# anitasyang/Laplace-GNN

Measured on AMD Instinct MI355X. Metric: la.fit() samples/sec (GCN, KFAC), higher is better.
Workload: dtype f32; 1 GPU; arxiv-shaped 2-layer GCN, hessian_structure=kron (BASELINE configs[2]); num_nodes=169343, nnz=2501719, features=128, hidden=256, classes=40, n_train=90941, batch_size=10000, batches=10, parallelism=dp1 ((batch, class) units, contiguous balanced runs)

## Files before the change

### include/laplace_gnn_hip.h

```cpp
#ifndef LAPLACE_GNN_HIP_H
#define LAPLACE_GNN_HIP_H

#include <stdint.h>

#ifdef __cplusplus
extern "C" {
#endif

#define LGNN_ABI_VERSION 1

#if defined(__GNUC__)
#define LGNN_API __attribute__((visibility("default")))
#else
#define LGNN_API
#endif

#define LGNN_KIND_GCN 0
#define LGNN_KIND_SAGE 1

#define LGNN_ACT_RELU 0
#define LGNN_ACT_TANH 1

#define LGNN_NORM_NONE 0
#define LGNN_NORM_LAYER 1
// ... 25 lines not shown
LGNN_API int lgnn_is_symmetric(const lgnn_ctx* h);

LGNN_API int lgnn_export_adj(const lgnn_ctx* h, int64_t* rows, int64_t* cols, void* stream);
LGNN_API int lgnn_adj_to_edge_index(const lgnn_ctx* h, int64_t* edge_index_out, int64_t* num_out, void* stream);
LGNN_API int lgnn_update_adjacency(lgnn_ctx* h, const int64_t* rows, const int64_t* cols, const uint8_t* state,
                                   int64_t num_flips, void* stream);
LGNN_API int lgnn_export_propagation(const lgnn_ctx* h, int64_t* rows, int64_t* cols, float* vals, void* stream);

LGNN_API int lgnn_bind_model(lgnn_ctx* h, int num_layers, const int64_t* dims ,
                    const float* const* weights ,
                    const float* const* biases , const float* X,
                    int activation, int likelihood);
LGNN_API int lgnn_bind_extras(lgnn_ctx* h, const float* const* res_weights, const float* const* res_biases, int norm_kind,
                     const float* const* norm_weight, const float* const* norm_bias, const float* const* norm_mean,
                     const float* const* norm_var, float norm_eps);
LGNN_API int lgnn_invalidate(lgnn_ctx* h);
LGNN_API int64_t lgnn_device_bytes(const lgnn_ctx* h);
LGNN_API int lgnn_set_workspace_limit(lgnn_ctx* h, int64_t bytes);

LGNN_API int lgnn_forward(lgnn_ctx* h, const int64_t* idx, int64_t M, float* out , void* stream);
LGNN_API int lgnn_forward_all(lgnn_ctx* h, float* out , void* stream);

#define LGNN_SAMPLED_SOFTMAX 1u
LGNN_API int lgnn_sampled_forward(lgnn_ctx* h, const int64_t* idx, int64_t M, const float* theta ,
                                  int64_t S, uint32_t flags , float* out ,
                                  void* stream);

LGNN_API int lgnn_train_forward(lgnn_ctx* h, const int64_t* idx, int64_t M, const uint8_t* const* drop_masks ,
                                float drop_scale, float* out , void* stream);
LGNN_API int lgnn_train_backward(lgnn_ctx* h, const float* grad_out , float* const* grad_W, float* const* grad_b,
                                 float* const* grad_res_W, float* const* grad_res_b, float* const* grad_norm_w,
                                 float* const* grad_norm_b, void* stream);

LGNN_API int lgnn_kfac_accumulate(lgnn_ctx* h, const int64_t* idx, const void* y, int64_t M, int64_t n_train,
                         uint32_t flags, float* const* A_out ,
                         float* const* B_out , float* loss_out,
                         void* stream);

LGNN_API int lgnn_kfac_accumulate_classes(lgnn_ctx* h, const int64_t* idx, const void* y, int64_t M, int64_t n_train,
                                 uint32_t flags, int64_t class_begin, int64_t class_end,
                                 float* const* A_out, float* const* B_out, float* loss_out, void* stream);

LGNN_API int lgnn_kfac_accumulate_share(lgnn_ctx* h, const int64_t* idx, const void* y, int64_t M, int64_t n_train,
                               uint32_t flags, int64_t part_begin, int64_t part_end, int64_t part_count,
                               float* const* A_out, float* const* B_out, float* loss_out, void* stream);

LGNN_API int lgnn_kfac_accumulate_fisher(lgnn_ctx* h, const int64_t* idx, const void* y_seed, const void* y_loss, int64_t M,
                                int64_t n_train, uint32_t flags, float resid_scale, float b_scale, float* const* A_out,
                                float* const* B_out, float* loss_out, void* stream);
LGNN_API int lgnn_ef_accumulate(lgnn_ctx* h, const int64_t* idx, const void* y_seed, const void* y_loss, int64_t M,
                       float resid_scale, float scale, float* diag_out, float* full_out, float* grads_out,
                       float* loss_out, void* stream);

LGNN_API int lgnn_kfac_plan(int kind, int num_layers, const int64_t* dims , int64_t num_nodes, int64_t nnz,
                   int activation, uint32_t flags, int64_t workspace_limit, int64_t* out );

LGNN_API int lgnn_diag_accumulate(lgnn_ctx* h, const int64_t* idx, const void* y, int64_t M, uint32_t flags,
                         float* diag_out , float* loss_out, void* stream);

LGNN_API int lgnn_full_accumulate(lgnn_ctx* h, const int64_t* idx, const void* y, int64_t M, float* H_out, float* loss_out,
                         void* stream);

LGNN_API int lgnn_lastlayer_full_accumulate(lgnn_ctx* h, const int64_t* idx, const void* y, int64_t M,
                                   float* H_out, float* loss_out, void* stream);

LGNN_API int lgnn_lastlayer_features(lgnn_ctx* h, const int64_t* idx, int64_t M, float* phi_out, float* f_out, void* stream);

LGNN_API int lgnn_lastlayer_pairs_accumulate(lgnn_ctx* h, const int64_t* idx, const void* y, int64_t M, float* S_pairs,
                                    float* Sb_pairs, float* loss_out, void* stream);
LGNN_API int lgnn_lastlayer_pairs_place(lgnn_ctx* h, const float* S_pairs, const float* Sb_pairs, float* H_out, void* stream);

LGNN_API int lgnn_lastlayer_kron_accumulate(lgnn_ctx* h, const int64_t* idx, const void* y, int64_t M, int64_t n_train,
                                   uint32_t flags, float* A_out, float* B_out, float* Bb_out, float* loss_out, void* stream);
LGNN_API int lgnn_lastlayer_diag_accumulate(lgnn_ctx* h, const int64_t* idx, const void* y, int64_t M, float* diag_out,
                                   float* loss_out, void* stream);

LGNN_API int lgnn_check_async_errors(lgnn_ctx* h, void* stream);
LGNN_API int lgnn_peek_async_errors(lgnn_ctx* h);

LGNN_API int lgnn_kfac_batch_tag(lgnn_ctx* h, uint64_t tag);
LGNN_API int lgnn_batch_cache_drop(lgnn_ctx* h, uint64_t tag);
LGNN_API int lgnn_batch_cache_stats(const lgnn_ctx* h, int64_t* out);

LGNN_API int lgnn_enable_kernel_timing(lgnn_ctx* h, int enable);
LGNN_API int lgnn_kernel_timing_read(lgnn_ctx* h, int64_t* launches, double* total_ms, int64_t* planes);
LGNN_API int lgnn_kernel_timing_launches(lgnn_ctx* h, double* ms_out, int64_t capacity, int64_t* launches);

LGNN_API int lgnn_jacobians(lgnn_ctx* h, const int64_t* idx, int64_t M, float* J, float* f_out, void* stream);

LGNN_API int lgnn_jacobians_subset(lgnn_ctx* h, const int64_t* idx, int64_t M, const int64_t* subnet, int64_t S, float* J,
                          float* f_out, void* stream);
LGNN_API int lgnn_subnet_full_accumulate(lgnn_ctx* h, const int64_t* idx, const void* y, int64_t M, const int64_t* subnet,
                                int64_t S, float* H_out, float* loss_out, void* stream);

#define LGNN_GP_INDEPENDENT 1
#define LGNN_GP_MATCHED 2
#define LGNN_GP_FROM_JACOBIANS 4
LGNN_API int lgnn_gp_kernel(lgnn_ctx* h, const int64_t* idx_a, int64_t Ma, const int64_t* idx_b, int64_t Mb, int flags,
                            float* K, int64_t ldk, void* stream);
LGNN_API int lgnn_gp_jvp(lgnn_ctx* h, const int64_t* idx, int64_t M, const float* v, float* out, void* stream);

LGNN_API int lgnn_kfac_adjgrad_batch(lgnn_ctx* h, const int64_t* idx, const void* y, int64_t M, uint32_t flags,
                            const float* const* gamma_B , float loss_scale,
                            float* grad_P, float* out_bar, const int32_t* cand_a, const int32_t* cand_b, int64_t num_cand,
                            float* grad_cand, void* stream);
LGNN_API int lgnn_adjgrad_finish(lgnn_ctx* h, const float* out_bar, const float* const* gamma_A ,
                        float a_scale, float* grad_P, float* grad_adj, const int32_t* cand_a, const int32_t* cand_b,
                        int64_t num_cand, float* grad_cand, float* grad_cand_adj, void* stream);

LGNN_API int lgnn_diag_adjgrad_batch(lgnn_ctx* h, const int64_t* idx, const void* y, int64_t M, const float* gamma,
                            float loss_scale, float* grad_P, float* out_bar, float* h1_bar, float* e_bar,
                            const int32_t* cand_a, const int32_t* cand_b, int64_t num_cand, float* grad_cand, void* stream);
LGNN_API int lgnn_diag_adjgrad_finish(lgnn_ctx* h, const float* out_bar, const float* h1_bar, const float* e_bar, float* grad_P,
                             float* grad_adj, const int32_t* cand_a, const int32_t* cand_b, int64_t num_cand,
                             float* grad_cand, float* grad_cand_adj, void* stream);

LGNN_API int lgnn_full_adjgrad_batch(lgnn_ctx* h, const int64_t* idx, const void* y, int64_t M, const float* Gamma,
                            float loss_scale, float* grad_P, float* out_bar, float* h1_bar, float* e_bar,
                            const int32_t* cand_a, const int32_t* cand_b, int64_t num_cand, float* grad_cand, void* stream);
LGNN_API int lgnn_full_directions(lgnn_ctx* h, const int64_t* idx, int64_t M, const float* Gamma, float* K_out, float* R_out,
                         void* stream);

LGNN_API int lgnn_kfac_adjgrad_batch_dense(lgnn_ctx* h, const int64_t* idx, const void* y, int64_t M, uint32_t flags,
                                  const float* const* gamma_B , float loss_scale,
                                  float* out_bar, float* grad_adj_dense, void* stream);
LGNN_API int lgnn_adjgrad_finish_dense(lgnn_ctx* h, const float* out_bar, const float* const* gamma_A, float a_scale,
                              float* grad_adj_dense, void* stream);
LGNN_API int lgnn_diag_adjgrad_batch_dense(lgnn_ctx* h, const int64_t* idx, const void* y, int64_t M, const float* gamma,
                                  float loss_scale, float* out_bar, float* h1_bar, float* e_bar, float* grad_adj_dense,
                                  void* stream);
LGNN_API int lgnn_diag_adjgrad_finish_dense(lgnn_ctx* h, const float* out_bar, const float* h1_bar, const float* e_bar,
                                   float* grad_adj_dense, void* stream);

LGNN_API int lgnn_lora_threshold(lgnn_ctx* h, const int32_t* base_rowptr, const int32_t* base_col, const float* lora_A,
                                 const float* lora_B, int64_t r, float scaling, float threshold, int symmetric,
                                 int64_t* num_flips, void* stream);
LGNN_API int lgnn_lora_grad(lgnn_ctx* h, const float* grad_adj_dense, const float* lora_A, const float* lora_B, int64_t r,
                            float scaling, float* grad_A, float* grad_B, void* stream);

LGNN_API int lgnn_glm_variance(lgnn_ctx* h, const int64_t* idx, int64_t M, const float* QA0, const float* QB0, const float* S0,
                      const float* QA1, const float* S1, const float* QB1sq, const float* kappa, float* f_mu,
                      float* f_var_diag, void* stream);
LGNN_API int lgnn_glm_variance_mapped(lgnn_ctx* h, const int64_t* idx, int64_t M, const float* W1m, int64_t Cm,
                             const float* QA0, const float* QB0, const float* S0, const float* QA1, const float* S1,
                             const float* QB1sq, const float* kappa, float* f_mu, float* var_mapped, void* stream);

LGNN_API int lgnn_glm_variance_ext(lgnn_ctx* h, const int64_t* idx, int64_t M, const float* W1m, int64_t Cm,
                          const float* QA0, const float* QB0, const float* S0, const float* QA1, const float* S1,
                          const float* QB1sq, const float* kappa, const float* QAr, const float* QBr, const float* Sr,
                          float* f_mu, float* f_var, void* stream);

LGNN_API int lgnn_symeig_batched(float* A, int64_t n, int64_t batch, float* W, int32_t* info, void* stream);

LGNN_API int lgnn_knn(const float* X, int64_t N, int64_t F, int64_t ld, int k, int32_t* nbr, float* dist,
                      int64_t* num_fallback, void* stream);

#ifdef __cplusplus
}
#endif
#endif
```

### laplace-gnn_amd/_lib.py

```python
from __future__ import annotations

import ctypes as C
import os

_HERE = os.path.dirname(os.path.abspath(__file__))
LIB_PATH = os.path.join(_HERE, os.environ.get("LGNN_LIB_DIR", "lib"), "liblaplace_gnn_hip.so")

KIND_GCN, KIND_SAGE = 0, 1
ACT_RELU, ACT_TANH = 0, 1
LIK_CLASSIFICATION, LIK_REGRESSION = 0, 1
NORM_NONE, NORM_LAYER, NORM_BATCH = 0, 1, 2
FLAG_FORK_EXACT_SEED, FLAG_NO_FUSE, FLAG_NO_PATHS, FLAG_FORCE_PATHS = 1, 2, 4, 8
GP_INDEPENDENT, GP_MATCHED, GP_FROM_JACOBIANS = 1, 2, 4
SAMPLED_SOFTMAX = 1

_vp, _i64, _i32, _u32 = C.c_void_p, C.c_int64, C.c_int, C.c_uint32
_pp = C.POINTER(C.c_void_p)
SIGNATURES = {
    "lgnn_abi_version": (_i32, []),
    "lgnn_last_error": (C.c_char_p, []),
    "lgnn_create": (_i32, [_pp, _i64, _vp, _i64, _i32, _i32, _vp]),
    "lgnn_destroy": (None, [_vp]),
    "lgnn_nnz": (_i64, [_vp]),
    "lgnn_num_nodes": (_i64, [_vp]),
    "lgnn_is_symmetric": (_i32, [_vp]),
    "lgnn_num_long_rows": (_i64, [_vp]),
    "lgnn_kfac_last_route": (_i32, [_vp]),
    "lgnn_kfac_last_top": (_i32, [_vp]),
    "lgnn_kfac_last_top_kernel": (_i32, [_vp]),
    "lgnn_export_adj": (_i32, [_vp, _vp, _vp, _vp]),
    "lgnn_update_adjacency": (_i32, [_vp, _vp, _vp, _vp, _i64, _vp]),
    "lgnn_adj_to_edge_index": (_i32, [_vp, _vp, C.POINTER(_i64), _vp]),
    "lgnn_export_propagation": (_i32, [_vp, _vp, _vp, _vp, _vp]),
    "lgnn_bind_model": (_i32, [_vp, _i32, C.POINTER(_i64), _pp, _pp, _vp, _i32, _i32]),
    "lgnn_bind_extras": (_i32, [_vp, _pp, _pp, _i32, _pp, _pp, _pp, _pp, C.c_float]),
    "lgnn_invalidate": (_i32, [_vp]),
    "lgnn_device_bytes": (_i64, [_vp]),
    "lgnn_set_workspace_limit": (_i32, [_vp, _i64]),
    "lgnn_forward": (_i32, [_vp, _vp, _i64, _vp, _vp]),
    "lgnn_forward_all": (_i32, [_vp, _vp, _vp]),
    "lgnn_sampled_forward": (_i32, [_vp, _vp, _i64, _vp, _i64, _u32, _vp, _vp]),
    "lgnn_train_forward": (_i32, [_vp, _vp, _i64, _pp, C.c_float, _vp, _vp]),
    "lgnn_train_backward": (_i32, [_vp, _vp, _pp, _pp, _pp, _pp, _pp, _pp, _vp]),
    "lgnn_kfac_accumulate": (_i32, [_vp, _vp, _vp, _i64, _i64, _u32, _pp, _pp, _vp, _vp]),
    "lgnn_kfac_accumulate_classes": (_i32, [_vp, _vp, _vp, _i64, _i64, _u32, _i64, _i64, _pp, _pp, _vp, _vp]),
    "lgnn_kfac_accumulate_share": (_i32, [_vp, _vp, _vp, _i64, _i64, _u32, _i64, _i64, _i64, _pp, _pp, _vp, _vp]),
    "lgnn_kfac_accumulate_fisher": (_i32, [_vp, _vp, _vp, _vp, _i64, _i64, _u32, C.c_float, C.c_float, _pp, _pp, _vp, _vp]),
    "lgnn_ef_accumulate": (_i32, [_vp, _vp, _vp, _vp, _i64, C.c_float, C.c_float, _vp, _vp, _vp, _vp, _vp]),
    "lgnn_kfac_plan": (_i32, [_i32, _i32, C.POINTER(_i64), _i64, _i64, _i32, _u32, _i64, C.POINTER(_i64)]),
    "lgnn_diag_accumulate": (_i32, [_vp, _vp, _vp, _i64, _u32, _vp, _vp, _vp]),
    "lgnn_full_accumulate": (_i32, [_vp, _vp, _vp, _i64, _vp, _vp, _vp]),
    "lgnn_lastlayer_full_accumulate": (_i32, [_vp, _vp, _vp, _i64, _vp, _vp, _vp]),
    "lgnn_lastlayer_features": (_i32, [_vp, _vp, _i64, _vp, _vp, _vp]),
    "lgnn_lastlayer_pairs_accumulate": (_i32, [_vp, _vp, _vp, _i64, _vp, _vp, _vp, _vp]),
    "lgnn_lastlayer_pairs_place": (_i32, [_vp, _vp, _vp, _vp, _vp]),
    "lgnn_lastlayer_kron_accumulate": (_i32, [_vp, _vp, _vp, _i64, _i64, _u32, _vp, _vp, _vp, _vp, _vp]),
    "lgnn_lastlayer_diag_accumulate": (_i32, [_vp, _vp, _vp, _i64, _vp, _vp, _vp]),
    "lgnn_check_async_errors": (_i32, [_vp, _vp]),
    "lgnn_peek_async_errors": (_i32, [_vp]),
    "lgnn_kfac_batch_tag": (_i32, [_vp, C.c_uint64]),
    "lgnn_batch_cache_drop": (_i32, [_vp, C.c_uint64]),
    "lgnn_batch_cache_stats": (_i32, [_vp, C.POINTER(_i64)]),
    "lgnn_enable_kernel_timing": (_i32, [_vp, _i32]),
    "lgnn_kernel_timing_read": (_i32, [_vp, C.POINTER(_i64), C.POINTER(C.c_double), C.POINTER(_i64)]),
    "lgnn_kernel_timing_launches": (_i32, [_vp, _vp, _i64, _vp]),
    "lgnn_kfac_adjgrad_batch": (_i32, [_vp, _vp, _vp, _i64, _u32, _pp, C.c_float, _vp, _vp, _vp, _vp, _i64, _vp, _vp]),
    "lgnn_adjgrad_finish": (_i32, [_vp, _vp, _pp, C.c_float, _vp, _vp, _vp, _vp, _i64, _vp, _vp, _vp]),
    "lgnn_diag_adjgrad_batch": (_i32, [_vp, _vp, _vp, _i64, _vp, C.c_float, _vp, _vp, _vp, _vp, _vp, _vp, _i64, _vp, _vp]),
    "lgnn_diag_adjgrad_finish": (_i32, [_vp, _vp, _vp, _vp, _vp, _vp, _vp, _vp, _i64, _vp, _vp, _vp]),
    "lgnn_full_adjgrad_batch": (_i32, [_vp, _vp, _vp, _i64, _vp, C.c_float, _vp, _vp, _vp, _vp, _vp, _vp, _i64, _vp, _vp]),
    "lgnn_full_directions": (_i32, [_vp, _vp, _i64, _vp, _vp, _vp, _vp]),
    "lgnn_kfac_adjgrad_batch_dense": (_i32, [_vp, _vp, _vp, _i64, _u32, _pp, C.c_float, _vp, _vp, _vp]),
    "lgnn_adjgrad_finish_dense": (_i32, [_vp, _vp, _pp, C.c_float, _vp, _vp]),
    "lgnn_diag_adjgrad_batch_dense": (_i32, [_vp, _vp, _vp, _i64, _vp, C.c_float, _vp, _vp, _vp, _vp, _vp]),
    "lgnn_diag_adjgrad_finish_dense": (_i32, [_vp, _vp, _vp, _vp, _vp, _vp]),
    "lgnn_lora_threshold": (_i32, [_vp, _vp, _vp, _vp, _vp, _i64, C.c_float, C.c_float, _i32, C.POINTER(_i64), _vp]),
    "lgnn_lora_grad": (_i32, [_vp, _vp, _vp, _vp, _i64, C.c_float, _vp, _vp, _vp]),
    "lgnn_glm_variance": (_i32, [_vp, _vp, _i64, _vp, _vp, _vp, _vp, _vp, _vp, _vp, _vp, _vp, _vp]),
    "lgnn_glm_variance_mapped": (_i32, [_vp, _vp, _i64, _vp, _i64, _vp, _vp, _vp, _vp, _vp, _vp, _vp, _vp, _vp, _vp]),
    "lgnn_glm_variance_ext": (_i32, [_vp, _vp, _i64, _vp, _i64, _vp, _vp, _vp, _vp, _vp, _vp, _vp, _vp, _vp, _vp, _vp, _vp,
                                     _vp]),
    "lgnn_symeig_batched": (_i32, [_vp, _i64, _i64, _vp, _vp, _vp]),
    "lgnn_jacobians": (_i32, [_vp, _vp, _i64, _vp, _vp, _vp]),
    "lgnn_jacobians_subset": (_i32, [_vp, _vp, _i64, _vp, _i64, _vp, _vp, _vp]),
    "lgnn_subnet_full_accumulate": (_i32, [_vp, _vp, _vp, _i64, _vp, _i64, _vp, _vp, _vp]),
    "lgnn_gp_kernel": (_i32, [_vp, _vp, _i64, _vp, _i64, _i32, _vp, _i64, _vp]),
    "lgnn_gp_jvp": (_i32, [_vp, _vp, _i64, _vp, _vp, _vp]),
    "lgnn_knn": (_i32, [_vp, _i64, _i64, _i64, _i32, _vp, _vp, C.POINTER(_i64), _vp]),
}

_lib = None


class HipLibraryError(RuntimeError):
    pass


def load():
    global _lib
    if _lib is not None:
        return _lib
    if not os.path.exists(LIB_PATH):
        raise HipLibraryError(
            f"{LIB_PATH} is missing: build it with `python -c 'import __graft_entry__ as g; g.build()'` "
            "(or `make -C laplace-gnn_amd/csrc`).  There is no CPU fallback."
        )
    lib = C.CDLL(LIB_PATH)
    for name, (res, args) in SIGNATURES.items():
        fn = getattr(lib, name)
        fn.restype, fn.argtypes = res, args
    if lib.lgnn_abi_version() != 1:
        raise HipLibraryError("ABI version mismatch between _lib.py and liblaplace_gnn_hip.so")
    _lib = lib
    return lib


def check(rc: int, what: str):
    if rc != 0:
        msg = load().lgnn_last_error().decode("utf-8", "replace")
        raise HipLibraryError(f"{what} failed (rc={rc}): {msg}")


def ptr_array(ptrs):
    arr = (C.c_void_p * len(ptrs))(*ptrs)
    return arr
```

### laplace-gnn_amd/csrc/eigh.hip

```cpp
#include <cstdio>

#include <rocsolver/rocsolver.h>

#include "gram256.h"
#include "lgnn_internal.h"

namespace lgnn {
namespace {
rocblas_handle g_handle = nullptr;
rocblas_handle g_eig_handle = nullptr;
struct EighScratch {
  DevBuf e_large;
  DevBuf e;
  DevBuf v;
  DevBuf tau;
  DevBuf d;
  DevBuf z;
  DevBuf info;
};
EighScratch& scratch() {
  static auto* s = new EighScratch;
  return *s;
}

constexpr int kBranches = 8;
rocblas_handle g_bh[kBranches] = {};
hipStream_t g_side[kBranches] = {};
hipEvent_t g_fork = nullptr, g_join[kBranches] = {};
constexpr int TN = 256;

__device__ __forceinline__ float wsum64(float v) {
#pragma unroll
  for (int o = 32; o > 0; o >>= 1) v += __shfl_xor(v, o);
  return v;
}

__global__ __launch_bounds__(1024) void tridiag256_kernel(const float* __restrict__ A, int n, float* __restrict__ D,
                                                          float* __restrict__ E, float* __restrict__ V,
                                                          float* __restrict__ tau, int nfull, int off, int vld) {
  __shared__ __attribute__((aligned(16))) float xs[TN], vs[TN], ps[TN], ws[TN];
  const int tid = threadIdx.x, lane = tid & 63, r = tid >> 2, q = tid & 3;
  const int64_t b = blockIdx.x;
  const float* __restrict__ Ab = A + b * int64_t(nfull) * nfull + int64_t(off) * nfull + off;
  float* __restrict__ Db = D + b * int64_t(nfull) + off;
  float* __restrict__ Eb = E + b * int64_t(nfull) + off;
  float* __restrict__ Vb = V + b * int64_t(nfull) * vld + int64_t(off) * vld + off;
  float* __restrict__ tb = tau + b * int64_t(nfull) + off;
  float a[64];
#pragma unroll
  for (int g = 0; g < 16; ++g)
#pragma unroll
    for (int i = 0; i < 4; ++i) {
      const int c = 16 * g + 4 * q + i;
      a[4 * g + i] = (r < n && c < n) ? Ab[int64_t(r) * nfull + c] : 0.f;
    }
  for (int k = 0; k < n - 1; ++k) {
    const int g0 = (k + 1) >> 4;
    if (r == k) {
#pragma unroll
      for (int g = 0; g < 16; ++g)
        *reinterpret_cast<float4*>(&xs[16 * g + 4 * q]) = make_float4(a[4 * g], a[4 * g + 1], a[4 * g + 2], a[4 * g + 3]);
    }
    __syncthreads();
    float sg = 0.f;
#pragma unroll
    for (int j = 0; j < 4; ++j) {
      const int c = lane + 64 * j;
      const float x = xs[c];
      sg += c > k + 1 ? x * x : 0.f;
    }
    sg = wsum64(sg);
    const float alpha = xs[k + 1];
    if (tid == 0) Db[k] = xs[k];
    if (sg == 0.f) {
      if (tid == 0) { Eb[k] = alpha; tb[k] = 0.f; }
      __syncthreads();
      continue;
    }
    const float nrm = sqrtf(alpha * alpha + sg);
    const float beta = alpha >= 0.f ? -nrm : nrm;
    const float t = (beta - alpha) / beta;
    const float inv = 1.f / (alpha - beta);
    if (tid < TN) {
      const float v = tid <= k ? 0.f : (tid == k + 1 ? 1.f : xs[tid] * inv);
      vs[tid] = v;
      Vb[int64_t(k) * vld + tid] = v;
    }
    if (tid == 0) { Eb[k] = beta; tb[k] = t; }
    __syncthreads();
    if (r > k) {
      float part = 0.f;
#pragma unroll
      for (int g = 0; g < 16; ++g)
        if (g >= g0) {
          const float4 v4 = *reinterpret_cast<const float4*>(&vs[16 * g + 4 * q]);
          part = fmaf(a[4 * g], v4.x, part); part = fmaf(a[4 * g + 1], v4.y, part);
          part = fmaf(a[4 * g + 2], v4.z, part); part = fmaf(a[4 * g + 3], v4.w, part);
        }
      part += __shfl_xor(part, 1);
      part += __shfl_xor(part, 2);
      if (q == 0) ps[r] = t * part;
    } else if (q == 0) {
      ps[r] = 0.f;
    }
    __syncthreads();
    float ds = 0.f;
#pragma unroll
    for (int j = 0; j < 4; ++j) ds += ps[lane + 64 * j] * vs[lane + 64 * j];
    ds = wsum64(ds);
    const float hd = 0.5f * t * ds;
    if (tid < TN) ws[tid] = ps[tid] - hd * vs[tid];
    __syncthreads();
    if (r > k) {
      const float vr = vs[r], wr = ws[r];
#pragma unroll
      for (int g = 0; g < 16; ++g)
        if (g >= g0) {
          const float4 v4 = *reinterpret_cast<const float4*>(&vs[16 * g + 4 * q]);
          const float4 w4 = *reinterpret_cast<const float4*>(&ws[16 * g + 4 * q]);
          a[4 * g] -= vr * w4.x + wr * v4.x; a[4 * g + 1] -= vr * w4.y + wr * v4.y;
          a[4 * g + 2] -= vr * w4.z + wr * v4.z; a[4 * g + 3] -= vr * w4.w + wr * v4.w;
        }
    }
  }
  if (r == n - 1) {
#pragma unroll
    for (int g = 0; g < 16; ++g)
      *reinterpret_cast<float4*>(&xs[16 * g + 4 * q]) = make_float4(a[4 * g], a[4 * g + 1], a[4 * g + 2], a[4 * g + 3]);
  }
  __syncthreads();
  if (tid == 0) { Db[n - 1] = xs[n - 1]; Eb[n - 1] = 0.f; tb[n - 1] = 0.f; }
}

__global__ __launch_bounds__(256) void backtransform_kernel(const float* __restrict__ Z, int n, const float* __restrict__ V,
                                                            const float* __restrict__ tau, const float* __restrict__ lam,
                                                            const int32_t* __restrict__ info_in, float* __restrict__ out,
                                                            float* __restrict__ W, int32_t* __restrict__ info) {
  const int lane = threadIdx.x & 63;
  const int j = blockIdx.x * 4 + (threadIdx.x >> 6);
  const int64_t b = blockIdx.y;
  if (j >= n) return;
  if (lane == 0) {
    W[b * n + j] = lam[b * n + j];
    if (j == 0) info[b] = info_in[b];
  }
  const float* __restrict__ zr = Z + (b * n + j) * int64_t(n);
  float* __restrict__ orow = out + (b * n + j) * int64_t(n);
  const float* __restrict__ Vb = V + b * int64_t(n) * TN;
  const float* __restrict__ tb = tau + b * int64_t(n);
  float z[4];
#pragma unroll
  for (int i = 0; i < 4; ++i) z[i] = 4 * lane + i < n ? zr[4 * lane + i] : 0.f;
  for (int k = n - 2; k >= 0; --k) {
    const float t = tb[k];
    if (t == 0.f) continue;
    const float4 v = *reinterpret_cast<const float4*>(Vb + int64_t(k) * TN + 4 * lane);
    float d = v.x * z[0] + v.y * z[1] + v.z * z[2] + v.w * z[3];
    d = wsum64(d) * t;
    z[0] -= d * v.x; z[1] -= d * v.y; z[2] -= d * v.z; z[3] -= d * v.w;
  }
#pragma unroll
  for (int i = 0; i < 4; ++i)
    if (4 * lane + i < n) orow[4 * lane + i] = z[i];
}

constexpr int SNB = 32;
constexpr int SRG = 8;
__global__ __launch_bounds__(1024) void tridiag_stream_kernel(float* __restrict__ A, int n, int ncols, float* __restrict__ D,
                                                              float* __restrict__ E, float* __restrict__ V,
                                                              float* __restrict__ tau) {
// ... 40 lines not shown
        const float x = c < n ? xs[c] : 0.f;
        sg += c > k + 1 ? x * x : 0.f;
      }
      sg = wsum64(sg);
      const float alpha = xs[k + 1];
      float t = 0.f, beta = alpha, inv = 0.f;
      if (sg != 0.f) {
        const float nrm = sqrtf(alpha * alpha + sg);
        beta = alpha >= 0.f ? -nrm : nrm;
        t = (beta - alpha) / beta;
        inv = 1.f / (alpha - beta);
      }
      if (tid < n) {
        const float v = (sg == 0.f || tid <= k) ? 0.f : (tid == k + 1 ? 1.f : xs[tid] * inv);
        vs[tid] = v;
        Vp[j * n + tid] = v;
        Vb[int64_t(k) * n + tid] = v;
      }
      if (tid == 0) { Db[k] = xs[k]; Eb[k] = beta; tb[k] = t; }
      __syncthreads();
      if (sg == 0.f) {
        if (tid < n) Wp[j * n + tid] = 0.f;
        __syncthreads();
        continue;
      }
      {
        float4 acc = make_float4(0.f, 0.f, 0.f, 0.f);
        if (c4 + 3 > k && c4 < n) {
          int r = k + 1 + rg;
          for (; r + 7 * SRG < n; r += 8 * SRG) {
            float4 a[8];
#pragma unroll
            for (int u = 0; u < 8; ++u) a[u] = *reinterpret_cast<const float4*>(Ab + int64_t(r + u * SRG) * n + c4);
#pragma unroll
            for (int u = 0; u < 8; ++u) {
              const float vv = vs[r + u * SRG];
              acc.x += a[u].x * vv; acc.y += a[u].y * vv; acc.z += a[u].z * vv; acc.w += a[u].w * vv;
            }
          }
          for (; r < n; r += SRG) {
            const float4 a0 = *reinterpret_cast<const float4*>(Ab + int64_t(r) * n + c4);
            const float v0 = vs[r];
            acc.x += a0.x * v0; acc.y += a0.y * v0; acc.z += a0.z * v0; acc.w += a0.w * v0;
          }
        }
        if (c4 < n) *reinterpret_cast<float4*>(pp + rg * n + c4) = acc;
        for (int i = wave; i < j; i += 16) {
          float s1 = 0.f, s2 = 0.f;
          for (int q = 0; q < per_lane; ++q) {
            const int c = lane + 64 * q;
            if (c < n) { const float v = vs[c]; s1 += Wp[i * n + c] * v; s2 += Vp[i * n + c] * v; }
          }
          s1 = wsum64(s1); s2 = wsum64(s2);
          if (lane == 0) { tv[i] = s1; tw[i] = s2; }
        }
      }
      __syncthreads();
      if (tid < n) {
        float p = 0.f;
        if (tid > k) {
#pragma unroll
          for (int g = 0; g < SRG; ++g) p += pp[g * n + tid];
          float p2 = 0.f;
#pragma unroll 4
          for (int i = 0; i < j; ++i) {
            p -= Vp[i * n + tid] * tv[i];
            p2 += Wp[i * n + tid] * tw[i];
          }
          p -= p2;
        }
        ps[tid] = t * p;
      }
      __syncthreads();
      float ds = 0.f;
      for (int q = 0; q < per_lane; ++q) {
        const int c = lane + 64 * q;
        if (c < n) ds += ps[c] * vs[c];
      }
      ds = wsum64(ds);
      const float hd = 0.5f * t * ds;
      if (tid < n) Wp[j * n + tid] = ps[tid] - hd * vs[tid];
      __syncthreads();
    }
    const int kb = k0 + jn;
    if (jn < SNB) {
      for (int q = tid; q < (SNB - jn) * n; q += 1024) { Vp[jn * n + q] = 0.f; Wp[jn * n + q] = 0.f; }
      __syncthreads();
    }
    {
      const int base = kb & ~31;
      const int nt = (n - base + 31) >> 5;
      const int l31 = lane & 31, lhi = lane >> 5;
      for (int tile = wave; tile < nt * nt; tile += 16) {
        const int tr = tile / nt, tc = tile - tr * nt;
        const int row = base + 32 * tr + l31, col = base + 32 * tc + l31;
        const int rr = row < n ? row : n - 1, cc = col < n ? col : n - 1;
        f32x16 acc;
#pragma unroll
        for (int q = 0; q < 16; ++q) acc[q] = 0.f;
#pragma unroll 8
        for (int kk = 0; kk < SNB / 2; ++kk) {
          const int i = 2 * kk + lhi;
          acc = __builtin_amdgcn_mfma_f32_32x32x2f32(Vp[i * n + rr], Wp[i * n + cc], acc, 0, 0, 0);
          acc = __builtin_amdgcn_mfma_f32_32x32x2f32(Wp[i * n + rr], Vp[i * n + cc], acc, 0, 0, 0);
        }
        if (col < n) {
#pragma unroll
          for (int q = 0; q < 16; ++q) {
            const int r = base + 32 * tr + (q & 3) + 8 * (q >> 2) + 4 * lhi;
            if (r < n) Ab[int64_t(r) * n + col] -= acc[q];
          }
        }
      }
    }
    __syncthreads();
  }
}

__global__ __launch_bounds__(256) void backtransform512_kernel(const float* __restrict__ Z, int n, const float* __restrict__ V,
                                                               const float* __restrict__ tau, const float* __restrict__ lam,
                                                               const int32_t* __restrict__ info_in, float* __restrict__ out,
                                                               float* __restrict__ W, int32_t* __restrict__ info) {
  const int lane = threadIdx.x & 63;
  const int j = blockIdx.x * 4 + (threadIdx.x >> 6);
  const int64_t b = blockIdx.y;
  if (j >= n) return;
  if (lane == 0) {
    W[b * n + j] = lam[b * n + j];
    if (j == 0) info[b] = info_in[b];
  }
  const float* __restrict__ zr = Z + (b * n + j) * int64_t(n);
  float* __restrict__ orow = out + (b * n + j) * int64_t(n);
  const float* __restrict__ Vb = V + b * int64_t(n) * n;
  const float* __restrict__ tb = tau + b * int64_t(n);
  const bool hi = 256 + 4 * lane < n;
  const bool lo = 4 * lane < n;
  float4 z0 = lo ? *reinterpret_cast<const float4*>(zr + 4 * lane) : make_float4(0.f, 0.f, 0.f, 0.f);
  float4 z1 = hi ? *reinterpret_cast<const float4*>(zr + 256 + 4 * lane) : make_float4(0.f, 0.f, 0.f, 0.f);
  for (int k = n - 2; k >= 0; --k) {
    const float t = tb[k];
    if (t == 0.f) continue;
    const float* __restrict__ vk = Vb + int64_t(k) * n;
    const float4 v0 = lo ? *reinterpret_cast<const float4*>(vk + 4 * lane) : make_float4(0.f, 0.f, 0.f, 0.f);
    const float4 v1 = hi ? *reinterpret_cast<const float4*>(vk + 256 + 4 * lane) : make_float4(0.f, 0.f, 0.f, 0.f);
    float d = v0.x * z0.x + v0.y * z0.y + v0.z * z0.z + v0.w * z0.w + v1.x * z1.x + v1.y * z1.y + v1.z * z1.z + v1.w * z1.w;
    d = wsum64(d) * t;
    z0.x -= d * v0.x; z0.y -= d * v0.y; z0.z -= d * v0.z; z0.w -= d * v0.w;
    z1.x -= d * v1.x; z1.y -= d * v1.y; z1.z -= d * v1.z; z1.w -= d * v1.w;
  }
  if (lo) *reinterpret_cast<float4*>(orow + 4 * lane) = z0;
  if (hi) *reinterpret_cast<float4*>(orow + 256 + 4 * lane) = z1;
}

int stedc_branch(int br, int branches, int64_t n, int64_t batch, hipStream_t st) {
  if (rocblas_set_stream(g_bh[br], st) != rocblas_status_success) { set_error("rocblas_set_stream failed"); return 3; }
  for (int64_t b = br; b < batch; b += branches) {
    const rocblas_status rs = rocsolver_sstedc(g_bh[br], rocblas_evect_tridiagonal, rocblas_int(n), scratch().d.as<float>() + b * n,
                                               scratch().e.as<float>() + b * n, scratch().z.as<float>() + b * n * n, rocblas_int(n),
                                               scratch().info.as<int32_t>() + b);
    if (rs != rocblas_status_success) { set_error("rocsolver_sstedc failed"); return 3; }
  }
  return 0;
}

int stedc_all(int64_t n, int64_t batch, hipStream_t s) {
  const int branches = int(std::min<int64_t>(batch, kBranches));
  for (int i = 0; i < branches; ++i) {
    if (!g_bh[i] && rocblas_create_handle(&g_bh[i]) != rocblas_status_success) { set_error("rocblas_create_handle failed"); return 3; }
    if (i > 0 && !g_side[i]) LGNN_HIP_CHECK(hipStreamCreateWithFlags(&g_side[i], hipStreamNonBlocking));
    if (!g_join[i]) LGNN_HIP_CHECK(hipEventCreateWithFlags(&g_join[i], hipEventDisableTiming));
  }
  if (!g_fork) LGNN_HIP_CHECK(hipEventCreateWithFlags(&g_fork, hipEventDisableTiming));
  if (branches == 1) {
    for (int i = 0; i < branches; ++i) LGNN_CALL(stedc_branch(i, branches, n, batch, s));
    return 0;
  }
  LGNN_HIP_CHECK(hipEventRecord(g_fork, s));
  for (int i = 0; i < branches; ++i) {
    hipStream_t st = i == 0 ? s : g_side[i];
    if (i > 0) LGNN_HIP_CHECK(hipStreamWaitEvent(st, g_fork, 0));
    LGNN_CALL(stedc_branch(i, branches, n, batch, st));
    if (i > 0) {
      LGNN_HIP_CHECK(hipEventRecord(g_join[i], st));
      LGNN_HIP_CHECK(hipStreamWaitEvent(s, g_join[i], 0));
    }
  }
  return 0;
}
}
}

namespace lgnn {
void* blas_handle(hipStream_t s) {
  if (!g_handle && rocblas_create_handle(&g_handle) != rocblas_status_success) return nullptr;
  if (rocblas_set_stream(g_handle, s) != rocblas_status_success) return nullptr;
  return g_handle;
}
}

using namespace lgnn;

extern "C" int lgnn_symeig_batched(float* A, int64_t n, int64_t batch, float* W, int32_t* info, void* stream) {
  if (!A || !W || !info) { set_error("null argument"); return 2; }
  LGNN_REQUIRE(n > 0 && n <= 32768 && batch > 0 && batch <= 65535, "symeig: bad shape");
  hipStream_t s = static_cast<hipStream_t>(stream);
  if (n <= TN && n >= 2) {
    LGNN_CALL(scratch().e.reserve(size_t(batch) * n * 4));
    LGNN_CALL(scratch().v.reserve(size_t(batch) * n * TN * 4));
    LGNN_CALL(scratch().tau.reserve(size_t(batch) * n * 4));
    LGNN_CALL(scratch().d.reserve(size_t(batch) * n * 4));
    LGNN_CALL(scratch().z.reserve(size_t(batch) * n * n * 4));
    LGNN_CALL(scratch().info.reserve(size_t(batch) * 4));
    hipLaunchKernelGGL(tridiag256_kernel, dim3(unsigned(batch)), dim3(1024), 0, s, A, int(n), scratch().d.as<float>(),
                       scratch().e.as<float>(), scratch().v.as<float>(), scratch().tau.as<float>(), int(n), 0, TN);
    LGNN_HIP_CHECK(hipGetLastError());
    LGNN_CALL(stedc_all(n, batch, s));
    hipLaunchKernelGGL(backtransform_kernel, dim3(unsigned(cdiv(n, 4)), unsigned(batch)), dim3(256), 0, s, scratch().z.as<float>(),
                       int(n), scratch().v.as<float>(), scratch().tau.as<float>(), scratch().d.as<float>(), scratch().info.as<int32_t>(), A, W, info);
    LGNN_HIP_CHECK(hipGetLastError());
    return 0;
  }
  if (n > TN && n <= 2 * TN && n % 4 == 0) {
    LGNN_CALL(scratch().e.reserve(size_t(batch) * n * 4));
    LGNN_CALL(scratch().v.reserve(size_t(batch) * n * n * 4));
    LGNN_CALL(scratch().tau.reserve(size_t(batch) * n * 4));
    LGNN_CALL(scratch().d.reserve(size_t(batch) * n * 4));
    LGNN_CALL(scratch().z.reserve(size_t(batch) * n * n * 4));
    LGNN_CALL(scratch().info.reserve(size_t(batch) * 4));
    const size_t smem = size_t(2 * SNB * n + SRG * n + 3 * n + 2 * SNB) * 4;
    LGNN_REQUIRE(smem <= 160 * 1024, "symeig: panel does not fit the LDS");
    static bool attr_set = false;
    if (!attr_set) {
      LGNN_HIP_CHECK(hipFuncSetAttribute(reinterpret_cast<const void*>(&tridiag_stream_kernel),
                                         hipFuncAttributeMaxDynamicSharedMemorySize, 160 * 1024));
      attr_set = true;
    }
    LGNN_HIP_CHECK(hipMemsetAsync(scratch().v.p, 0, size_t(batch) * n * n * 4, s));
    hipLaunchKernelGGL(tridiag_stream_kernel, dim3(unsigned(batch)), dim3(1024), smem, s, A, int(n), int(n - TN),
                       scratch().d.as<float>(), scratch().e.as<float>(), scratch().v.as<float>(), scratch().tau.as<float>());
    hipLaunchKernelGGL(tridiag256_kernel, dim3(unsigned(batch)), dim3(1024), 0, s, A, TN, scratch().d.as<float>(), scratch().e.as<float>(),
                       scratch().v.as<float>(), scratch().tau.as<float>(), int(n), int(n - TN), int(n));
    LGNN_HIP_CHECK(hipGetLastError());
    LGNN_CALL(stedc_all(n, batch, s));
    hipLaunchKernelGGL(backtransform512_kernel, dim3(unsigned(cdiv(n, 4)), unsigned(batch)), dim3(256), 0, s, scratch().z.as<float>(),
                       int(n), scratch().v.as<float>(), scratch().tau.as<float>(), scratch().d.as<float>(), scratch().info.as<int32_t>(), A, W, info);
    LGNN_HIP_CHECK(hipGetLastError());
    return 0;
  }
  if (!g_eig_handle && rocblas_create_handle(&g_eig_handle) != rocblas_status_success) { set_error("rocBLAS handle"); return 3; }
  if (rocblas_set_stream(g_eig_handle, s) != rocblas_status_success) { set_error("rocBLAS stream setup failed"); return 3; }
  LGNN_CALL(scratch().e_large.reserve(size_t(batch) * n * 4));
  const rocblas_status st = rocsolver_ssyevd_strided_batched(
      g_eig_handle, rocblas_evect_original, rocblas_fill_upper, rocblas_int(n), A, rocblas_int(n), rocblas_stride(n * n), W,
      rocblas_stride(n), scratch().e_large.as<float>(), rocblas_stride(n), info, rocblas_int(batch));
  if (st != rocblas_status_success) { set_error("rocsolver_ssyevd_strided_batched failed"); return 3; }
  return 0;
}
```

Baseline: 2.500 million samples/s.

## Replace rocSOLVER stedc with a fused batched divide-and-conquer tridiagonal eigensolver kernel

Adds a single-block-per-matrix GPU kernel that solves the symmetric tridiagonal eigenproblem by divide-and-conquer. It handles deflation and Givens rotations, solves the secular equation by bisection, and builds eigenvector updates with MFMA. It replaces the per-matrix rocsolver_sstedc calls spread over side streams inside symeig for n up to 256, so launch and handle overhead go away. In exchange it adds a second n×n ping-pong scratch buffer, and accuracy now depends on bisection-based eigenvalues and single-precision deflation tolerances.

```diff
diff --git a/include/laplace_gnn_hip.h b/include/laplace_gnn_hip.h
--- a/include/laplace_gnn_hip.h
+++ b/include/laplace_gnn_hip.h
@@ -201,6 +201,8 @@
 
 LGNN_API int lgnn_symeig_batched(float* A, int64_t n, int64_t batch, float* W, int32_t* info, void* stream);
 
+LGNN_API int lgnn_tridiag_eig(float* d, float* e, int64_t n, int64_t batch, float* Z, int32_t* info, void* stream);
+
 LGNN_API int lgnn_knn(const float* X, int64_t N, int64_t F, int64_t ld, int k, int32_t* nbr, float* dist,
                       int64_t* num_fallback, void* stream);
 
diff --git a/laplace-gnn_amd/_lib.py b/laplace-gnn_amd/_lib.py
--- a/laplace-gnn_amd/_lib.py
+++ b/laplace-gnn_amd/_lib.py
@@ -81,6 +81,7 @@
     "lgnn_glm_variance_ext": (_i32, [_vp, _vp, _i64, _vp, _i64, _vp, _vp, _vp, _vp, _vp, _vp, _vp, _vp, _vp, _vp, _vp, _vp,
                                      _vp]),
     "lgnn_symeig_batched": (_i32, [_vp, _i64, _i64, _vp, _vp, _vp]),
+    "lgnn_tridiag_eig": (_i32, [_vp, _vp, _i64, _i64, _vp, _vp, _vp]),
     "lgnn_jacobians": (_i32, [_vp, _vp, _i64, _vp, _vp, _vp]),
     "lgnn_jacobians_subset": (_i32, [_vp, _vp, _i64, _vp, _i64, _vp, _vp, _vp]),
     "lgnn_subnet_full_accumulate": (_i32, [_vp, _vp, _vp, _i64, _vp, _i64, _vp, _vp, _vp]),
diff --git a/laplace-gnn_amd/csrc/eigh.hip b/laplace-gnn_amd/csrc/eigh.hip
--- a/laplace-gnn_amd/csrc/eigh.hip
+++ b/laplace-gnn_amd/csrc/eigh.hip
@@ -16,6 +16,7 @@
   DevBuf tau;
   DevBuf d;
   DevBuf z;
+  DevBuf z2;
   DevBuf info;
 };
 EighScratch& scratch() {
@@ -362,6 +363,441 @@
   if (hi) *reinterpret_cast<float4*>(orow + 256 + 4 * lane) = z1;
 }
 
+constexpr int DCN = 256;
+constexpr float DC_EPS = 5.9604645e-8f;
+constexpr int DC_BISECT = 32;
+
+struct DcNode { int lo, hi, mid; };
+__device__ __forceinline__ DcNode dc_node(int node, int k, int n) {
+  return {(node * n) >> k, ((node + 1) * n) >> k, ((2 * node + 1) * n) >> (k + 1)};
+}
+__device__ __forceinline__ float quad_sum(float v) {
+  v += __shfl_xor(v, 1);
+  v += __shfl_xor(v, 2);
+  return v;
+}
+
+template <int C, int R>
+__device__ __forceinline__ void dc_secular(bool active, int lo, int q, int kk, float rho, int sub, const float* __restrict__ dsv,
+                                           const float* __restrict__ z2n, const float* __restrict__ d2n,
+                                           float* __restrict__ mu, float* __restrict__ lam, float* __restrict__ dov, int g) {
+  float dr[4 * R], zr[4 * R];
+  const bool last = q == kk - 1;
+  const float dj = active ? dsv[lo + q] : 0.f;
+  const float dn = (active && !last) ? dsv[lo + q + 1] : dj;
+  const float gap = last ? rho : dn - dj;
+  const float half = 0.5f * gap;
+  float dorg = dj;
+  auto load = [&]() {
+#pragma unroll
+    for (int c = 0; c < R; ++c)
+#pragma unroll
+      for (int i = 0; i < 4; ++i) {
+        const int t = 16 * c + 4 * sub + i;
+        dr[4 * c + i] = (active && t < kk) ? dsv[lo + t] - dorg : 1e30f;
+      }
+  };
+  auto eval = [&](float m) {
+    float s = 0.f;
+#pragma unroll
+    for (int c = 0; c < 4 * R; ++c) s = fmaf(zr[c], __builtin_amdgcn_rcpf(dr[c] - m), s);
+#pragma unroll
+    for (int c = R; c < C; ++c) {
+      const float4 zz = *reinterpret_cast<const float4*>(z2n + 16 * c + 4 * sub);
+      const float4 dd = *reinterpret_cast<const float4*>(d2n + 16 * c + 4 * sub);
+      s = fmaf(zz.x, __builtin_amdgcn_rcpf((dd.x - dorg) - m), s);
+      s = fmaf(zz.y, __builtin_amdgcn_rcpf((dd.y - dorg) - m), s);
+      s = fmaf(zz.z, __builtin_amdgcn_rcpf((dd.z - dorg) - m), s);
+      s = fmaf(zz.w, __builtin_amdgcn_rcpf((dd.w - dorg) - m), s);
+    }
+    return 1.f + rho * quad_sum(s);
+  };
+#pragma unroll
+  for (int c = 0; c < R; ++c) {
+    const float4 zz = *reinterpret_cast<const float4*>(z2n + 16 * c + 4 * sub);
+    zr[4 * c] = zz.x; zr[4 * c + 1] = zz.y; zr[4 * c + 2] = zz.z; zr[4 * c + 3] = zz.w;
+  }
+  load();
+  const bool left = last || eval(half) > 0.f;
+  if (!left) { dorg = dn; load(); }
+  float a = left ? 0.f : -half, b = left ? half : 0.f;
+  if (last) b = gap;
+  for (int it = 0; it < DC_BISECT; ++it) {
+    if (C > R) asm volatile("" ::: "memory");
+    const float m = 0.5f * (a + b);
+    if (m == a || m == b) break;
+    const bool pos = eval(m) > 0.f;
+    b = pos ? m : b;
+    a = pos ? a : m;
+  }
+  if (active && sub == 0) {
+    const float m = 0.5f * (a + b);
+    mu[g] = m;
+    lam[g] = dorg + m;
+    dov[g] = dorg;
+  }
+}
+
+__global__ __launch_bounds__(1024) void tridiag_dc_kernel(float* __restrict__ D, const float* __restrict__ E, int n,
+                                                          float* __restrict__ Z, float* __restrict__ Zalt,
+                                                          int32_t* __restrict__ info) {
+  __shared__ float Dc[DCN], es[DCN], zv[DCN], Ds[DCN], zs[DCN], dsv[DCN], zsv[DCN], mu[DCN], lam[DCN], zh[DCN], invn[DCN], dov[DCN], Dd[DCN];
+  __shared__ float rc[DCN], rs[DCN];
+  __shared__ int nodeof[DCN];
+  __shared__ int srow[DCN], sv[DCN], dl[DCN], l1[DCN], l2[DCN], typ[DCN], svrow[DCN], rpj[DCN], rnj[DCN];
+  __shared__ __attribute__((aligned(16))) float z2a[2048], d2a[2048];
+  __shared__ float n_rho[DCN / 2], n_tol[DCN / 2];
+  __shared__ int n_k[DCN / 2], n_k1[DCN / 2], n_k2[DCN / 2], n_flag[DCN / 2], n_nrot[DCN / 2];
+  __shared__ int bad;
+  const int tid = threadIdx.x, lane = tid & 63, wave = tid >> 6;
+  const int64_t bi = blockIdx.x;
+  float* __restrict__ Db = D + bi * n;
+  const float* __restrict__ Eb = E + bi * n;
+  float* bufs[2] = {Z + bi * int64_t(n) * n, Zalt + bi * int64_t(n) * n};
+  if (tid == 0) bad = 0;
+  if (tid < DCN) {
+    srow[tid] = 0; sv[tid] = 0; dl[tid] = 0; l1[tid] = 0; l2[tid] = 0; typ[tid] = 0; svrow[tid] = 0;
+    rpj[tid] = 0; rnj[tid] = 0;
+  }
+  __syncthreads();
+  if (tid < n) {
+    const float d = Db[tid], e = tid < n - 1 ? Eb[tid] : 0.f;
+    if (!(fabsf(d) <= 3.0e38f) || !(fabsf(e) <= 3.0e38f)) bad = 1;
+    es[tid] = e;
+  }
+  __syncthreads();
+  if (bad) {
+    if (tid == 0) info[bi] = 1;
+    return;
+  }
+  if (tid < n) Dc[tid] = Db[tid] - (tid > 0 ? fabsf(es[tid - 1]) : 0.f) - (tid < n - 1 ? fabsf(es[tid]) : 0.f);
+  for (int r = wave; r < n; r += 16)
+    for (int c = lane; c < n; c += 64) {
+      const float v = r == c ? 1.f : 0.f;
+      bufs[0][int64_t(r) * n + c] = v;
+      bufs[1][int64_t(r) * n + c] = v;
+    }
+  int L = 0;
+  while ((1 << L) < n) ++L;
+  int cur = (L + 1) & 1;
+  __syncthreads();
+
+  for (int k = L - 1; k >= 0; --k) {
+    const int nodes = 1 << k;
+    const int mmax = (n + nodes - 1) >> k;
+    int stride = 16;
+    while (stride < mmax) stride <<= 1;
+    float* __restrict__ src = bufs[cur];
+    float* __restrict__ dst = bufs[cur ^ 1];
+    const int t = tid;
+    int node = 0;
+    DcNode nd = {0, 0, 0};
+    bool mine = false;
+    if (t < n) {
+      node = (((t + 1) << k) - 1) / n;
+      nd = dc_node(node, k, n);
+      mine = nd.hi - nd.lo >= 2;
+      nodeof[t] = node;
+    }
+    const int lo = nd.lo, mid = nd.mid;
+    if (mine) {
+      const float e = es[mid - 1];
+      zv[t] = t < mid ? src[int64_t(t) * n + mid - 1] : (e >= 0.f ? 1.f : -1.f) * src[int64_t(t) * n + mid];
+    }
+    if (tid < nodes) { n_flag[tid] = 0; n_nrot[tid] = 0; n_k[tid] = 0; }
+    for (int q = tid; q < nodes * stride; q += 1024) { z2a[q] = 0.f; d2a[q] = 1e30f; }
+    __syncthreads();
+    {
+      const int g = tid >> 2, sub = tid & 3;
+      int gnode = 0;
+      DcNode b = {0, 0, 0};
+      if (g < n) {
+        gnode = (((g + 1) << k) - 1) / n;
+        b = dc_node(gnode, k, n);
+      }
+      const bool gmine = b.hi - b.lo >= 2;
+      float nrm2 = 0.f, zmax = 0.f, dmax = 0.f;
+#pragma unroll 4
+      for (int j = b.lo + sub; j < b.hi; j += 4) {
+        const float zz = zv[j];
+        nrm2 = fmaf(zz, zz, nrm2);
+        zmax = fmaxf(zmax, fabsf(zz));
+        dmax = fmaxf(dmax, fabsf(Dc[j]));
+      }
+      nrm2 = quad_sum(nrm2);
+      zmax = fmaxf(zmax, __shfl_xor(zmax, 1)); zmax = fmaxf(zmax, __shfl_xor(zmax, 2));
+      dmax = fmaxf(dmax, __shfl_xor(dmax, 1)); dmax = fmaxf(dmax, __shfl_xor(dmax, 2));
+      const float inv = nrm2 > 0.f ? 1.f / sqrtf(nrm2) : 0.f;
+      const float rho = gmine ? fabsf(es[b.mid - 1]) * nrm2 * (inv > 0.f ? 1.f : 0.f) : 0.f;
+      const float gtol = 8.f * DC_EPS * fmaxf(dmax, zmax * inv);
+      const float myz = gmine ? zv[g] * inv : 0.f, myD = gmine ? Dc[g] : 0.f;
+      const bool mytiny = !(rho * fabsf(myz) > gtol);
+      int rank = 0, kq = 0, ktot = 0, q1 = 0, k1tot = 0;
+#pragma unroll 4
+      for (int j = b.lo + sub; j < b.hi; j += 4) {
+        const float Dj = Dc[j];
+        const bool before = Dj < myD || (Dj == myD && j < g);
+        const bool keep = rho * fabsf(zv[j] * inv) > gtol;
+        rank += before;
+        kq += before && keep;
+        ktot += keep;
+        q1 += before && keep && j < b.mid;
+        k1tot += keep && j < b.mid;
+      }
+      rank += __shfl_xor(rank, 1); rank += __shfl_xor(rank, 2);
+      kq += __shfl_xor(kq, 1); kq += __shfl_xor(kq, 2);
+      ktot += __shfl_xor(ktot, 1); ktot += __shfl_xor(ktot, 2);
+      q1 += __shfl_xor(q1, 1); q1 += __shfl_xor(q1, 2);
+      k1tot += __shfl_xor(k1tot, 1); k1tot += __shfl_xor(k1tot, 2);
+      if (gmine && sub == 0) {
+        const int p = b.lo + rank;
+        Ds[p] = myD; zs[p] = myz; srow[p] = g; typ[p] = g < b.mid ? 1 : 2;
+        if (!mytiny) {
+          sv[b.lo + kq] = p;
+          if (g < b.mid) l1[b.lo + q1] = kq; else l2[b.lo + kq - q1] = kq;
+        } else {
+          dl[b.lo + rank - kq] = p;
+          Dd[b.lo + rank - kq] = myD;
+        }
+        if (g == b.lo) { n_rho[gnode] = rho; n_tol[gnode] = gtol; n_k[gnode] = ktot; n_k1[gnode] = k1tot; n_k2[gnode] = ktot - k1tot; }
+      }
+    }
+    __syncthreads();
+    if (mine) {
+      const int q = t - lo;
+      if (q >= 1 && q < n_k[node]) {
+        const int p = sv[lo + q], pp = sv[lo + q - 1];
+        const float s = zs[pp], c = zs[p], tt = Ds[p] - Ds[pp];
+        if (fabsf(tt * c * s) <= n_tol[node] * (c * c + s * s)) n_flag[node] = 1;
+      }
+    }
+    __syncthreads();
+    const int any = __syncthreads_or(tid < nodes && n_flag[tid] != 0);
+    if (any) {
+      if (tid < nodes && n_flag[tid]) {
+        const DcNode b = dc_node(tid, k, n);
+        const float rho = n_rho[tid], btol = n_tol[tid];
+        int ks = 0, k1 = 0, k2 = 0, ndef = 0, nr = 0, prev = -1, typrev = 0;
+        float zprev = 0.f, dprev = 0.f;
+        auto emit = [&]() {
+          sv[b.lo + ks] = prev; dsv[b.lo + ks] = dprev; zsv[b.lo + ks] = zprev;
+          if (typrev & 1) l1[b.lo + k1++] = ks;
+          if (typrev & 2) l2[b.lo + k2++] = ks;
+          ++ks;
+        };
+#pragma unroll 4
+        for (int p = b.lo; p < b.hi; ++p) {
+          const float zp = zs[p], dp = Ds[p];
+          const int tp = typ[p];
+          if (!(rho * fabsf(zp) > btol)) { dl[b.lo + ndef] = p; Dd[b.lo + ndef] = dp; ++ndef; continue; }
+          if (prev >= 0) {
+            const float tt = dp - dprev, tau2 = zp * zp + zprev * zprev;
+            if (fabsf(tt * zp * zprev) <= btol * tau2) {
+              const float tau = sqrtf(tau2), c = zp / tau, s = -zprev / tau;
+              rpj[b.lo + nr] = prev; rnj[b.lo + nr] = p; rc[b.lo + nr] = c; rs[b.lo + nr] = s; ++nr;
+              dl[b.lo + ndef] = prev; Dd[b.lo + ndef] = dprev * c * c + dp * s * s; ++ndef;
+              dprev = dprev * s * s + dp * c * c;
+              zprev = tau;
+              typrev = typrev != tp ? 3 : tp;
+              prev = p;
+              continue;
+            }
+            emit();
+          }
+          prev = p; zprev = zp; dprev = dp; typrev = tp;
+        }
+        if (prev >= 0) emit();
+        n_k[tid] = ks; n_k1[tid] = k1; n_k2[tid] = k2; n_nrot[tid] = nr;
+      }
+      __syncthreads();
+      if (mine) {
+        const int nr = n_nrot[node];
+        float carry = 0.f;
+        int last = -1;
+        for (int r0 = 0; r0 < nr; r0 += 4) {
+          float x[4], y[4];
+          int pj[4], nj[4];
+#pragma unroll
+          for (int u = 0; u < 4; ++u) {
+            const int r = min(r0 + u, nr - 1);
+            pj[u] = rpj[lo + r]; nj[u] = rnj[lo + r];
+            x[u] = src[int64_t(srow[pj[u]]) * n + t];
+            y[u] = src[int64_t(srow[nj[u]]) * n + t];
+          }
+#pragma unroll
+          for (int u = 0; u < 4; ++u) {
+            if (r0 + u < nr) {
+              const float c = rc[lo + r0 + u], sn = rs[lo + r0 + u];
+              float xx = x[u];
+              if (pj[u] == last) xx = carry;
+              else if (last >= 0) src[int64_t(srow[last]) * n + t] = carry;
+              src[int64_t(srow[pj[u]]) * n + t] = c * xx + sn * y[u];
+              carry = c * y[u] - sn * xx;
+              last = nj[u];
+            }
+          }
+        }
+        if (last >= 0) src[int64_t(srow[last]) * n + t] = carry;
+      }
+      __syncthreads();
+    }
+    const int kk = mine ? n_k[node] : 0;
+    if (mine && t - lo < kk) {
+      const int p = sv[t];
+      const bool scanned = n_flag[node] != 0;
+      const float zz = scanned ? zsv[t] : zs[p], dd = scanned ? dsv[t] : Ds[p];
+      dsv[t] = dd; zsv[t] = zz; svrow[t] = srow[p];
+      z2a[node * stride + (t - lo)] = zz * zz;
+      d2a[node * stride + (t - lo)] = dd;
+    }
+    __syncthreads();
+    {
+      const int g = tid >> 2, sub = tid & 3;
+      int gnode = 0, glo = 0, gk = 0;
+      bool active = false;
+      if (g < n) {
+        gnode = (((g + 1) << k) - 1) / n;
+        const DcNode b = dc_node(gnode, k, n);
+        glo = b.lo;
+        gk = b.hi - b.lo >= 2 ? n_k[gnode] : 0;
+        active = g - glo < gk;
+      }
+      const float rho = active ? n_rho[gnode] : 0.f;
+      const float* z2n = z2a + (active ? gnode * stride : 0);
+      const float* d2n = d2a + (active ? gnode * stride : 0);
+      const int q = g - glo;
+      if (stride <= 16) dc_secular<1, 1>(active, glo, q, gk, rho, sub, dsv, z2n, d2n, mu, lam, dov, g);
+      else if (stride <= 32) dc_secular<2, 2>(active, glo, q, gk, rho, sub, dsv, z2n, d2n, mu, lam, dov, g);
+      else if (stride <= 64) dc_secular<4, 4>(active, glo, q, gk, rho, sub, dsv, z2n, d2n, mu, lam, dov, g);
+      else if (stride <= 128) dc_secular<8, 4>(active, glo, q, gk, rho, sub, dsv, z2n, d2n, mu, lam, dov, g);
+      else dc_secular<16, 4>(active, glo, q, gk, rho, sub, dsv, z2n, d2n, mu, lam, dov, g);
+      __syncthreads();
+      float prod = 1.f;
+      const float di = active ? dsv[g] : 0.f;
+#pragma unroll 4
+      for (int j = sub; j < (active ? gk : 0); j += 4) {
+        const float num = (dov[glo + j] - di) + mu[glo + j];
+        const float den = j == q ? 1.f : dsv[glo + j] - di;
+        prod *= num / den;
+      }
+      prod *= __shfl_xor(prod, 1);
+      prod *= __shfl_xor(prod, 2);
+      if (active && sub == 0) zh[g] = copysignf(sqrtf(fabsf(prod / rho)), zsv[g]);
+      __syncthreads();
+      float s2 = 0.f;
+      if (active) {
+        const float dorg = dov[g], mj = mu[g];
+#pragma unroll 4
+        for (int i = sub; i < gk; i += 4) {
+          const float u = zh[glo + i] / ((dsv[glo + i] - dorg) - mj);
+          s2 = fmaf(u, u, s2);
+        }
+      }
+      s2 = quad_sum(s2);
+      if (active && sub == 0) invn[g] = 1.f / sqrtf(s2);
+      __syncthreads();
+    }
+    {
+      const int l31 = lane & 31, lhi = lane >> 5;
+      auto do_tile = [&](const DcNode& b, int bk, int bk1, int bk2, int tr, int tc) {
+        const int c0 = b.lo + 32 * tc, c1 = min(c0 + 32, b.hi);
+        const int* list = nullptr;
+        int cnt = bk;
+        if (c1 <= b.mid) { list = l1 + b.lo; cnt = bk1; }
+        else if (c0 >= b.mid) { list = l2 + b.lo; cnt = bk2; }
+        const int j = 32 * tr + l31;
+        const bool rowok = j < bk;
+        const int jj = rowok ? j : 0;
+        const float dorg = dov[b.lo + jj], mj = mu[b.lo + jj], inj = rowok ? invn[b.lo + jj] : 0.f;
+        const int col = c0 + l31;
+        const bool colok = col < b.hi;
+        const int colc = colok ? col : b.hi - 1;
+        f32x16 acc;
+#pragma unroll
+        for (int q = 0; q < 16; ++q) acc[q] = 0.f;
+        for (int s = 0; s < cnt; s += 8) {
+          float av[4], bv[4];
+#pragma unroll
+          for (int u = 0; u < 4; ++u) {
+            const int idx = s + 2 * u + lhi;
+            const bool ok = idx < cnt;
+            const int ic = ok ? idx : 0;
+            const int qi = list ? list[ic] : ic;
+            const float bb = src[int64_t(svrow[b.lo + qi]) * n + colc];
+            const float aa = zh[b.lo + qi] * inj * __builtin_amdgcn_rcpf((dsv[b.lo + qi] - dorg) - mj);
+            av[u] = ok ? aa : 0.f;
+            bv[u] = (ok && colok) ? bb : 0.f;
+          }
+#pragma unroll
+          for (int u = 0; u < 4; ++u) acc = __builtin_amdgcn_mfma_f32_32x32x2f32(av[u], bv[u], acc, 0, 0, 0);
+        }
+        if (colok) {
+#pragma unroll
+          for (int q = 0; q < 16; ++q) {
+            const int r = 32 * tr + (q & 3) + 8 * (q >> 2) + 4 * lhi;
+            if (r < bk) dst[int64_t(b.lo + r) * n + col] = acc[q];
+          }
+        }
+      };
+      if (mmax <= 32) {
+        for (int nn = wave; nn < nodes; nn += 16) {
+          const DcNode b = dc_node(nn, k, n);
+          const int bk = b.hi - b.lo >= 2 ? n_k[nn] : 0;
+          if (bk > 0) do_tile(b, bk, bk, bk, 0, 0);
+        }
+      } else {
+        int item = 0;
+        for (int nn = 0; nn < nodes; ++nn) {
+          const DcNode b = dc_node(nn, k, n);
+          const int bk = n_k[nn], bk1 = n_k1[nn], bk2 = n_k2[nn];
+          const int rt = (bk + 31) >> 5, ct = (b.hi - b.lo + 31) >> 5;
+          for (int tile = 0; tile < rt * ct; ++tile, ++item)
+            if ((item & 15) == wave) do_tile(b, bk, bk1, bk2, tile / ct, tile % ct);
+        }
+      }
+      int sh = 4;
+      while ((1 << sh) < stride) ++sh;
+#pragma unroll 4
+      for (int idx = tid; idx < (n << sh); idx += 1024) {
+        const int g = idx >> sh, gnode = nodeof[g];
+        const DcNode b = dc_node(gnode, k, n);
+        const int c = b.lo + (idx & (stride - 1)), bk = n_k[gnode], q = g - b.lo;
+        if (b.hi - b.lo >= 2 && q >= bk && c < b.hi) dst[int64_t(g) * n + c] = src[int64_t(srow[dl[g - bk]]) * n + c];
+      }
+      if (mine) Dc[t] = t - lo < kk ? lam[t] : Dd[t - kk];
+    }
+    __syncthreads();
+    cur ^= 1;
+  }
+  {
+    const float* __restrict__ src = bufs[cur];
+    float* __restrict__ dst = bufs[cur ^ 1];
+    {
+      const int g = tid >> 2, sub = tid & 3;
+      const float myD = g < n ? Dc[g] : 0.f;
+      int rank = 0;
+#pragma unroll 4
+      for (int j = sub; j < n; j += 4) {
+        const float Dj = Dc[j];
+        rank += Dj < myD || (Dj == myD && j < g);
+      }
+      rank += __shfl_xor(rank, 1); rank += __shfl_xor(rank, 2);
+      if (g < n && sub == 0) { srow[rank] = g; Db[rank] = myD; }
+    }
+    __syncthreads();
+#pragma unroll 2
+    for (int r = wave; r < n; r += 16) {
+      const int sr = srow[r];
+#pragma unroll
+      for (int j = 0; j < 4; ++j) {
+        const int c = lane + 64 * j;
+        if (c < n) dst[int64_t(r) * n + c] = src[int64_t(sr) * n + c];
+      }
+    }
+    if (tid == 0) info[bi] = 0;
+  }
+}
+
 int stedc_branch(int br, int branches, int64_t n, int64_t batch, hipStream_t st) {
   if (rocblas_set_stream(g_bh[br], st) != rocblas_status_success) { set_error("rocblas_set_stream failed"); return 3; }
   for (int64_t b = br; b < batch; b += branches) {
@@ -409,6 +845,16 @@
 }
 
 using namespace lgnn;
+
+extern "C" int lgnn_tridiag_eig(float* d, float* e, int64_t n, int64_t batch, float* Z, int32_t* info, void* stream) {
+  if (!d || !e || !Z || !info) { set_error("null argument"); return 2; }
+  LGNN_REQUIRE(n > 0 && n <= DCN && batch > 0 && batch <= 65535, "tridiag_eig: bad shape");
+  hipStream_t s = static_cast<hipStream_t>(stream);
+  LGNN_CALL(scratch().z2.reserve(size_t(batch) * n * n * 4));
+  hipLaunchKernelGGL(tridiag_dc_kernel, dim3(unsigned(batch)), dim3(1024), 0, s, d, e, int(n), Z, scratch().z2.as<float>(), info);
+  LGNN_HIP_CHECK(hipGetLastError());
+  return 0;
+}
 
 extern "C" int lgnn_symeig_batched(float* A, int64_t n, int64_t batch, float* W, int32_t* info, void* stream) {
   if (!A || !W || !info) { set_error("null argument"); return 2; }
@@ -420,11 +866,14 @@
     LGNN_CALL(scratch().tau.reserve(size_t(batch) * n * 4));
     LGNN_CALL(scratch().d.reserve(size_t(batch) * n * 4));
     LGNN_CALL(scratch().z.reserve(size_t(batch) * n * n * 4));
+    LGNN_CALL(scratch().z2.reserve(size_t(batch) * n * n * 4));
     LGNN_CALL(scratch().info.reserve(size_t(batch) * 4));
     hipLaunchKernelGGL(tridiag256_kernel, dim3(unsigned(batch)), dim3(1024), 0, s, A, int(n), scratch().d.as<float>(),
                        scratch().e.as<float>(), scratch().v.as<float>(), scratch().tau.as<float>(), int(n), 0, TN);
     LGNN_HIP_CHECK(hipGetLastError());
-    LGNN_CALL(stedc_all(n, batch, s));
+    hipLaunchKernelGGL(tridiag_dc_kernel, dim3(unsigned(batch)), dim3(1024), 0, s, scratch().d.as<float>(), scratch().e.as<float>(),
+                       int(n), scratch().z.as<float>(), scratch().z2.as<float>(), scratch().info.as<int32_t>());
+    LGNN_HIP_CHECK(hipGetLastError());
     hipLaunchKernelGGL(backtransform_kernel, dim3(unsigned(cdiv(n, 4)), unsigned(batch)), dim3(256), 0, s, scratch().z.as<float>(),
                        int(n), scratch().v.as<float>(), scratch().tau.as<float>(), scratch().d.as<float>(), scratch().info.as<int32_t>(), A, W, info);
     LGNN_HIP_CHECK(hipGetLastError());
```

Result: faster. 2.560 million samples/s (median of 6 runs) (+2.4%).
